# TUMFTM/RadarGNN

Hardware: AMD Instinct MI355X
Metric: radar frames/sec (graph-build + GNN fwd) (higher is better)
Workload: dtype f32 (dense layers: fp32 operands split into 2 f16 terms after an exact power-of-two pre-scale, 3 f16 MFMA products per fp32 product, fp32 accumulate -- more accurate than fp32 MFMA against float64, tests/test_gpu_f16x2.py; RGNN_NO_F16X2=1 selects 3 bf16 terms / 6 products, RGNN_LINEAR_FP32=1 v_mfma_; 1 GPU; C2: per GPU 64 RadarScenes-shaped frames x 3000 pts, radius graph r=1.0, node feats [rcs,velocity_vector,time_index,degree], edge feats [relative_position], 4-layer MPNNConv [224,224,128,64] + emb MLPs + both heads, train-mode BatchNorm, max aggr; frames_per_gpu=64, points_per_gpu=192000, edges_per_gpu=799078, ranks_in_process_group=1

## Files before the change

### include/rgnn.h

```cpp
#ifndef RGNN_H
#define RGNN_H

#include <stdint.h>

#ifdef __cplusplus
extern "C" {
#endif

typedef void* rgnn_stream_t;

#define RGNN_OK 0
#define RGNN_ERR_INVALID_ARGUMENT (-1)
#define RGNN_ERR_LAUNCH (-2)
#define RGNN_ERR_UNSUPPORTED (-3)

#define RGNN_STATUS_KNN_TOO_FEW_POINTS 1
#define RGNN_STATUS_DOT_PRODUCT 2
#define RGNN_STATUS_TIME_INDEX_OVERFLOW 4
#define RGNN_STATUS_EDGE_COUNT_CHANGED 8
#define RGNN_STATUS_NOT_SYMMETRIC 16
#define RGNN_STATUS_SPLITK_TIMEOUT 32
#define RGNN_STATUS_GT_OBJECT_TOO_LARGE 64
#define RGNN_STATUS_GT_DEGENERATE_OBJECT 128
#define RGNN_STATUS_PREPROCESS_BAD_ROW 256
// ... 120 lines not shown
int rgnn_radius_counts(const int32_t* deg, int64_t n, const int32_t* rowptr, int32_t threshold, int32_t* out2, rgnn_stream_t stream);

#define RGNN_STAT_ROWS 4
#define RGNN_AFFINE_ROWS 3
typedef struct rgnn_linear_args {
  const float* A1; int64_t lda1; int32_t k1;
  const float* A2; int64_t lda2; int32_t k2;
  const float* W1; const float* W2; int64_t ldw; int32_t w_split;
  const float* bias1; const float* bias2;
  const float* residual; int64_t ldr;
  float* out; int64_t ldo;
  int64_t m; int32_t n;
  int32_t relu_out;
  float* col_stats;
  const int32_t* row_index;
  const int64_t* m_dev;
  int32_t accumulate;
  int32_t gather_only;
  const int32_t* residual_index;
  const void* W_planes;
  int32_t w_planes_kp;
  void* splitk_ws;
  int64_t splitk_ws_bytes;
  const float* a1_scale_shift;
  int32_t a1_relu;
  int32_t relu_from_col;
  const void* W_planes_f16;
  const float* a1_bound;
  const float* a2_bound;
  float* out_absmax;
  const int32_t* a1_panel_segment;
} rgnn_linear_args;
#define RGNN_BOUND_SLOTS 256
enum { RGNN_LINEAR_PATH_OTHER = 0, RGNN_LINEAR_PATH_DMA_BF16X3 = 1, RGNN_LINEAR_PATH_DMA_F16X2 = 2 };
int32_t rgnn_linear_fwd_path(const rgnn_linear_args* args );
int64_t rgnn_linear_planes_f16_bytes(int32_t n, int32_t k);
int rgnn_linear_split_weights_f16(const float* W1, const float* W2, int64_t ldw, int32_t w_split, int32_t n, int32_t k,
                                  void* planes , rgnn_stream_t stream);
int32_t rgnn_linear_fwd_fuses_a1_affine(const rgnn_linear_args* args );
enum { RGNN_LINEAR_FAMILY_NONE = 0, RGNN_LINEAR_FAMILY_TINY = 1, RGNN_LINEAR_FAMILY_FP32 = 2, RGNN_LINEAR_FAMILY_X3 = 3,
       RGNN_LINEAR_FAMILY_DMA = 4 };
void rgnn_linear_fwd_plan(const rgnn_linear_args* args , int32_t out[8] );
int64_t rgnn_linear_splitk_ws_bytes(void);
int64_t rgnn_linear_stat_panels(int64_t m);
int32_t rgnn_linear_planes_kp(int32_t k);
int rgnn_linear_split_weights(const float* W1, const float* W2, int64_t ldw, int32_t w_split, int32_t n, int32_t k,
                              void* planes , rgnn_stream_t stream);
int rgnn_linear_fwd(const rgnn_linear_args* args , rgnn_stream_t stream);

int32_t rgnn_embed3_supported(int32_t k0, int32_t n1, int32_t n2, int32_t n3);
int rgnn_embed3(const float* x, int64_t ldx, int32_t k0, const float* W1, int64_t ldw1, const float* b1, int32_t n1,
                const void* W2_planes_f16, const float* b2, int32_t n2, const void* W3_planes_f16, const float* b3, int32_t n3,
                int32_t relu3, int64_t m, float* out, int64_t ldo, float* out_absmax, rgnn_stream_t stream);
int rgnn_tiny_mlp2(const float* A, int64_t lda, int32_t k0, const int32_t* row_index , int64_t m,
                   const float* W1, int64_t ldw1, const float* b1, int32_t n1, int32_t relu1, const float* W2, int64_t ldw2,
                   const float* b2, int32_t n2, int32_t relu2, float* out, int64_t ldo, rgnn_stream_t stream);

int rgnn_batchnorm_finalize(const float* stats_a, int64_t panels_a, const int64_t* rows_a ,
                            const float* stats_b , int64_t panels_b, const int64_t* rows_b ,
                            int64_t m, int32_t n, const float* gamma, const float* beta, float* running_mean,
                            float* running_var, int64_t* num_batches_tracked, int32_t training, float momentum, float eps,
                            float* scale_shift , const float* in_bound ,
                            float* out_bound , rgnn_stream_t stream);
int rgnn_batchnorm_segments(const float* x, int64_t ldx, const int64_t* seg_ptr , int64_t n_seg, int32_t n,
                            const float* gamma, const float* beta, float* running_mean, float* running_var,
                            int64_t* num_batches_tracked, float momentum, float eps, double* seg_sums, float* table,
                            const float* in_bound, float* out_bound, rgnn_stream_t stream);
int rgnn_batchnorm_act_segments(const float* x, int64_t ldx, const int64_t* seg_ptr, int64_t n_seg, int32_t n, const float* gamma,
                                const float* beta, float* running_mean, float* running_var, int64_t* num_batches_tracked,
                                float momentum, float eps, int32_t relu, double* seg_sums, float* table, float* y, int64_t ldy,
                                const float* in_bound, float* out_bound, rgnn_stream_t stream);
int rgnn_batchnorm_segments_from_panels(const float* stats_a, const int32_t* panel_start_a, const float* stats_b,
                                        const int32_t* panel_start_b, const int64_t* seg_ptr, int64_t n_seg, int32_t n,
                                        const float* gamma, const float* beta, float* running_mean, float* running_var,
                                        int64_t* num_batches_tracked, float momentum, float eps, double* seg_sums, float* table,
                                        const float* in_bound, float* out_bound, rgnn_stream_t stream);
int rgnn_pad_list_by_segment(const int32_t* list, const int64_t* count, const int64_t* seg_ptr, int64_t n_seg, int32_t* out_list,
                             int64_t* out_count, int32_t* tile_segment, int32_t* stat_panel_start, rgnn_stream_t stream);
int rgnn_pad_list_pair_by_segment(const int32_t* list_a, const int64_t* count_a, const int32_t* list_b, const int64_t* count_b,
                                  const int64_t* seg_ptr, int64_t n_seg, int32_t* out_list_a, int64_t* out_count_a,
                                  int32_t* tile_segment_a, int32_t* stat_panel_start_a, int32_t* out_list_b, int64_t* out_count_b,
                                  int32_t* tile_segment_b, int32_t* stat_panel_start_b, rgnn_stream_t stream);
int rgnn_scale_shift_act_segments(const float* x, int64_t ldx, const float* table, const int64_t* seg_ptr, int64_t n_seg,
                                  int64_t m, int32_t n, int32_t relu, float* y, int64_t ldy, rgnn_stream_t stream);
int rgnn_column_stats(const float* x, int64_t ldx, int64_t m, int32_t n, float* col_stats ,
                      rgnn_stream_t stream);
int rgnn_scale_shift_act(const float* x, int64_t ldx, const float* scale_shift, int64_t m, int32_t n, int32_t relu,
                         float* y, int64_t ldy, rgnn_stream_t stream);

#define RGNN_AGGR_MAX 0
#define RGNN_AGGR_MEAN 1
#define RGNN_AGGR_ADD 2
#define RGNN_AGGR_MIN 3
#define RGNN_AGGR_VAR 4
#define RGNN_AGGR_STD 5
#define RGNN_MPNN_SKIP_EMPTY_ROWS 1
int rgnn_mpnn_aggregate(const float* P, int64_t ldp, const float* p_bias, const float* Q, int64_t ldq,
                        const float* We , int64_t ldwe, const float* edge_attr_sorted,
                        int32_t de, const int32_t* rowptr_t, const int32_t* src_sorted,
                        const int32_t* node_order ,
                        const int32_t* chunk_start , int32_t n_chunks, int64_t n,
                        int32_t d, int32_t aggr, float* out, int64_t ldo, int32_t flags, float* out_absmax ,
                        rgnn_stream_t stream);
int rgnn_mpnn_aggregate_max_arg(const float* p_bias, const float* Q, int64_t ldq, const float* We, int64_t ldwe,
                                const float* edge_attr_sorted, int32_t de, const int32_t* rowptr_t, const int32_t* src_sorted,
                                const int32_t* node_order, const int32_t* chunk_start, int32_t n_chunks, int64_t n, int32_t d,
// ... 230 lines not shown
```

### radargnn_amd/_lib.py

```python
from __future__ import annotations

import ctypes as C
import os

import torch

_HERE = os.path.dirname(os.path.abspath(__file__))
LIB_PATH = os.environ.get("RGNN_LIB") or os.path.join(_HERE, "librgnn.so")

c_i32, c_i64, c_f32, c_f64, c_vp = C.c_int32, C.c_int64, C.c_float, C.c_double, C.c_void_p


class RgnnGrid(C.Structure):
    _fields_ = [("X", c_vp), ("dim", c_i32), ("n", c_i64), ("frame_ptr", c_vp), ("n_frames", c_i64),
                ("ws", c_vp), ("ws_bytes", c_i64)]


class RgnnLinearArgs(C.Structure):
    _fields_ = [("A1", c_vp), ("lda1", c_i64), ("k1", c_i32),
                ("A2", c_vp), ("lda2", c_i64), ("k2", c_i32),
                ("W1", c_vp), ("W2", c_vp), ("ldw", c_i64), ("w_split", c_i32),
                ("bias1", c_vp), ("bias2", c_vp),
                ("residual", c_vp), ("ldr", c_i64),
                ("out", c_vp), ("ldo", c_i64),
                ("m", c_i64), ("n", c_i32),
                ("relu_out", c_i32),
                ("col_stats", c_vp),
                ("row_index", c_vp), ("m_dev", c_vp), ("accumulate", c_i32), ("gather_only", c_i32),
                ("residual_index", c_vp),
                ("W_planes", c_vp), ("w_planes_kp", c_i32),
                ("splitk_ws", c_vp), ("splitk_ws_bytes", c_i64),
                ("a1_scale_shift", c_vp), ("a1_relu", c_i32), ("relu_from_col", c_i32),
                ("W_planes_f16", c_vp), ("a1_bound", c_vp), ("a2_bound", c_vp), ("out_absmax", c_vp), ("a1_panel_segment", c_vp)]


class RgnnEvalBoxes(C.Structure):
    _fields_ = [("translation", c_vp), ("size", c_vp), ("rotation", c_vp), ("velocity", c_vp), ("name", c_vp), ("attribute", c_vp),
                ("keep", c_vp), ("ptr", c_vp), ("n", c_i64)]


SIGNATURES = {
    "rgnn_version": (C.c_char_p, []),
    "rgnn_last_error": (C.c_char_p, []),
    "rgnn_env_reload": (None, []),
    "rgnn_profile_next_launch": (None, [c_vp, c_vp]),
    "rgnn_stream_create": (c_i32, [C.POINTER(c_vp)]),
    "rgnn_stream_destroy": (c_i32, [c_vp]),
    "rgnn_scan_tmp_bytes": (c_i64, [c_i64]),
    "rgnn_exclusive_scan_i32": (c_i32, [c_vp, c_vp, c_i64, c_vp, c_vp]),
    "rgnn_grid_workspace_bytes": (c_i64, [c_i64, c_i64, c_i32]),
    "rgnn_grid_build": (c_i32, [C.POINTER(RgnnGrid), c_f64, c_f64, c_i64, c_vp]),
    "rgnn_grid_order_offsets": (c_i32, [c_i64, c_i64, c_i32, C.POINTER(c_i64), C.POINTER(c_i64)]),
    "rgnn_radius_graph_count": (c_i32, [C.POINTER(RgnnGrid), c_f64, c_vp, c_vp]),
    "rgnn_radius_graph_fill": (c_i32, [C.POINTER(RgnnGrid), c_f64, c_vp, c_vp, c_vp, c_i64, c_vp, c_vp, c_vp]),
    "rgnn_radius_graph_rows": (c_i32, [C.POINTER(RgnnGrid), c_f64, c_vp, c_vp, c_vp, c_i64, c_vp, c_vp, c_vp, c_i32, c_vp]),
    "rgnn_radius_graph_rows_direct": (c_i32, [C.POINTER(RgnnGrid), c_f64, c_vp, c_vp, c_vp, c_i64, c_vp, c_vp, c_vp, c_i32, c_vp]),
    "rgnn_radius_rows_commit": (c_i32, [c_vp, c_i64, c_i64, c_vp, c_vp, c_vp, c_vp, c_vp]),
    "rgnn_knn_graph": (c_i32, [C.POINTER(RgnnGrid), c_i32, c_i64, c_vp, c_vp, c_vp, c_vp, c_i32, c_vp, c_vp]),
    "rgnn_knn_degree_from_csr": (c_i32, [c_vp, c_vp, c_vp, c_vp, c_i64, c_i32, c_vp, c_vp]),
    "rgnn_undirected_degree_preset": (c_i32, [c_vp, c_vp, c_i64, c_vp, c_vp]),
    "rgnn_grid_cell_order": (c_i32, [C.POINTER(RgnnGrid), c_vp, c_vp]),
    "rgnn_undirected_degree": (c_i32, [c_vp, c_vp, c_i64, c_vp, c_vp]),
    "rgnn_csr_by_target_tmp_bytes": (c_i64, [c_i64, c_i64]),
    "rgnn_invert_permutation": (c_i32, [c_vp, c_i64, c_vp, c_vp]),
    "rgnn_source_rowptr": (c_i32, [c_vp, c_i64, c_i64, c_vp, c_vp, c_vp, c_vp]),
    "rgnn_csr_by_target": (c_i32, [c_vp, c_i64, c_i64, c_vp, c_vp, c_vp, c_vp, c_vp, c_i32, c_vp]),
    "rgnn_csr_by_target_frames": (c_i32, [c_vp, c_i64, c_i64, c_i64, c_vp, c_i64, c_i64, c_vp, c_vp, c_vp, c_vp, c_vp, c_vp, c_vp, c_vp]),
    "rgnn_csr_by_target_symmetric": (c_i32, [c_vp, c_vp, c_i64, c_i64, c_vp, c_vp, c_vp, c_vp, c_vp, c_vp, c_vp, c_vp]),
    "rgnn_embed3_supported": (c_i32, [c_i32, c_i32, c_i32, c_i32]),
    "rgnn_embed3": (c_i32, [c_vp, c_i64, c_i32, c_vp, c_i64, c_vp, c_i32, c_vp, c_vp, c_i32, c_vp, c_vp, c_i32, c_i32, c_i64, c_vp, c_i64,
                            c_vp, c_vp]),
    "rgnn_edge_features": (c_i32, [c_vp, c_vp, c_vp, c_i64, C.POINTER(c_i32), c_i32, c_i32, c_vp, c_i32, c_vp, c_vp]),
    "rgnn_edge_features_reversed": (c_i32, [c_vp, c_vp, c_vp, c_i64, c_vp, c_i64, C.POINTER(c_i32), c_i32, c_i32, c_vp, c_i32, c_vp, c_vp]),
    "rgnn_node_features": (c_i32, [c_vp, c_vp, c_vp, c_vp, c_vp, c_i64, C.POINTER(c_i32), c_i32, c_vp, c_i32, c_vp]),
    "rgnn_node_features_time_index": (c_i32, [c_vp, c_vp, c_vp, c_vp, c_vp, c_i64, c_vp, c_i64, C.POINTER(c_i32), c_i32, c_vp, c_i32,
                                              c_vp, c_vp, c_vp]),
    "rgnn_split_by_degree_frames": (c_i32, [c_vp, c_vp, c_i64, c_vp, c_vp, c_vp, c_vp, c_vp, c_vp, c_vp]),
    "rgnn_radius_counts": (c_i32, [c_vp, c_i64, c_vp, c_i32, c_vp, c_vp]),
    "rgnn_time_index": (c_i32, [c_vp, c_vp, c_i64, c_vp, c_vp, c_vp]),
    "rgnn_time_index_ws_bytes": (c_i64, [c_i64]),
    "rgnn_time_index_ws": (c_i32, [c_vp, c_vp, c_i64, c_i64, c_vp, c_vp, c_vp, c_i64, c_vp]),
    "rgnn_linear_stat_panels": (c_i64, [c_i64]),
    "rgnn_linear_fwd": (c_i32, [C.POINTER(RgnnLinearArgs), c_vp]),
    "rgnn_linear_fwd_fuses_a1_affine": (c_i32, [C.POINTER(RgnnLinearArgs)]),
    "rgnn_linear_fwd_plan": (None, [C.POINTER(RgnnLinearArgs), C.POINTER(c_i32 * 8)]),
    "rgnn_linear_planes_kp": (c_i32, [c_i32]),
    "rgnn_linear_fwd_path": (c_i32, [C.POINTER(RgnnLinearArgs)]),
    "rgnn_linear_planes_f16_bytes": (c_i64, [c_i32, c_i32]),
    "rgnn_linear_split_weights_f16": (c_i32, [c_vp, c_vp, c_i64, c_i32, c_i32, c_i32, c_vp, c_vp]),
    "rgnn_linear_splitk_ws_bytes": (c_i64, []),
    "rgnn_linear_split_weights": (c_i32, [c_vp, c_vp, c_i64, c_i32, c_i32, c_i32, c_vp, c_vp]),
    "rgnn_tiny_mlp2": (c_i32, [c_vp, c_i64, c_i32, c_vp, c_i64, c_vp, c_i64, c_vp, c_i32, c_i32, c_vp, c_i64, c_vp, c_i32, c_i32, c_vp,
                       c_i64, c_vp]),
    "rgnn_batchnorm_finalize": (c_i32, [c_vp, c_i64, c_vp, c_vp, c_i64, c_vp, c_i64, c_i32, c_vp, c_vp, c_vp, c_vp, c_vp, c_i32, c_f32,
                                        c_f32, c_vp, c_vp, c_vp, c_vp]),
    "rgnn_batchnorm_segments": (c_i32, [c_vp, c_i64, c_vp, c_i64, c_i32, c_vp, c_vp, c_vp, c_vp, c_vp, c_f32, c_f32, c_vp, c_vp,
                                        c_vp, c_vp, c_vp]),
    "rgnn_batchnorm_act_segments": (c_i32, [c_vp, c_i64, c_vp, c_i64, c_i32, c_vp, c_vp, c_vp, c_vp, c_vp, c_f32, c_f32, c_i32, c_vp,
                                            c_vp, c_vp, c_i64, c_vp, c_vp, c_vp]),
    "rgnn_batchnorm_segments_from_panels": (c_i32, [c_vp, c_vp, c_vp, c_vp, c_vp, c_i64, c_i32, c_vp, c_vp, c_vp, c_vp, c_vp, c_f32,
                                                    c_f32, c_vp, c_vp, c_vp, c_vp, c_vp]),
    "rgnn_pad_list_by_segment": (c_i32, [c_vp, c_vp, c_vp, c_i64, c_vp, c_vp, c_vp, c_vp, c_vp]),
    "rgnn_pad_list_pair_by_segment": (c_i32, [c_vp, c_vp, c_vp, c_vp, c_vp, c_i64, c_vp, c_vp, c_vp, c_vp, c_vp, c_vp, c_vp, c_vp, c_vp]),
    "rgnn_scale_shift_act_segments": (c_i32, [c_vp, c_i64, c_vp, c_vp, c_i64, c_i64, c_i32, c_i32, c_vp, c_i64, c_vp]),
    "rgnn_column_stats": (c_i32, [c_vp, c_i64, c_i64, c_i32, c_vp, c_vp]),
    "rgnn_scale_shift_act": (c_i32, [c_vp, c_i64, c_vp, c_i64, c_i32, c_i32, c_vp, c_i64, c_vp]),
    "rgnn_mpnn_aggregate": (c_i32, [c_vp, c_i64, c_vp, c_vp, c_i64, c_vp, c_i64, c_vp, c_i32, c_vp, c_vp, c_vp, c_vp, c_i32, c_i64,
                                    c_i32, c_i32, c_vp, c_i64, c_i32, c_vp, c_vp]),
    "rgnn_mpnn_aggregate_max_arg": (c_i32, [c_vp, c_vp, c_i64, c_vp, c_i64, c_vp, c_i32, c_vp, c_vp, c_vp, c_vp, c_i32, c_i64, c_i32,
                                            c_vp, c_i64, c_vp, c_i32, C.POINTER(c_i32), c_vp, c_vp]),
    "rgnn_mpnn_win_plan_ints": (c_i64, [c_i64, c_i64]),
    "rgnn_mpnn_win_plan_counters": (None, [c_i64, c_i64, C.POINTER(c_i64), C.POINTER(c_i64)]),
    "rgnn_mpnn_win_plan": (c_i32, [c_vp, c_vp, c_vp, c_i64, c_i64, c_vp, c_vp]),
    "rgnn_mpnn_aggregate_win": (c_i32, [c_vp, c_vp, c_i64, c_vp, c_i64, c_vp, c_i32, c_vp, c_vp, c_vp, c_vp, c_i64, c_i64, c_i32, c_vp,
                                        c_i64, c_i32, c_vp, c_vp, c_vp]),
    "rgnn_mpnn_win_wplanes_bytes": (c_i64, [c_i32]),
    "rgnn_mpnn_win_wplanes": (c_i32, [c_vp, c_i64, c_i32, c_i32, c_vp, c_vp, c_vp]),
    "rgnn_empty_targets": (c_i32, [c_vp, c_vp, c_i64, c_vp, c_vp, c_vp, c_vp, c_vp, c_vp, c_vp]),
    "rgnn_split_targets": (c_i32, [c_vp, c_vp, c_i64, c_vp, c_vp, c_vp, c_vp, c_vp, c_vp, c_vp, c_vp, c_vp]),
    "rgnn_split_targets_by_node": (c_i32, [c_vp, c_vp, c_i64, c_vp, c_vp, c_vp, c_vp, c_vp, c_vp, c_vp, c_vp, c_vp]),
    "rgnn_mpnn_num_chunks": (c_i32, [c_i64, c_i64]),
    "rgnn_mpnn_work_units": (c_i32, [c_i64, c_i64]),
    "rgnn_mpnn_target_weight": (c_i32, [c_i64, c_i64]),
    "rgnn_mpnn_partition": (c_i32, [c_vp, c_i64, c_i64, c_vp, c_vp]),
# ... 105 lines not shown
```

### radargnn_amd/csrc/embed.hip

```cpp
#include "linear_common.h"

namespace {

typedef short raw16x8 __attribute__((ext_vector_type(8)));
constexpr int EM_THREADS = 512, EM_ROWS = 256;

__device__ __forceinline__ float wave_max(float v) {
#pragma unroll
  for (int o = 32; o > 0; o >>= 1) v = fmaxf(v, __shfl_xor(v, o, 64));
  return v;
}
__device__ __forceinline__ void prescale_of(float bound, float& a_mul, float& inv) {
  const int be = (int)((__float_as_uint(bound) >> 23) & 255u);
  int se = 268 - be;
  se = se > 253 ? 253 : se;
  a_mul = __uint_as_float((unsigned)se << 23);
  inv = __uint_as_float((unsigned)(254 - se) << 23);
}
__device__ __forceinline__ void split8(const float (&x)[8], float mul, raw16x8& h, raw16x8& l) {
  f16x8_t hh, ll;
#pragma unroll
  for (int i = 0; i < 8; i++) {
    const float v = x[i] * mul;
    const _Float16 a = (_Float16)v;
// ... 91 lines not shown
        my_stage[((r & 3) + 8 * (r >> 2) + 4 * half) * LDS2 + col] = v;
      }
    }
    m2 = wave_max(m2);
    float mul2, inv2;
    prescale_of(m2, mul2, inv2);
    __builtin_amdgcn_fence(__ATOMIC_ACQ_REL, "wavefront");
    __builtin_amdgcn_wave_barrier();
    f32x16 acc3[T3];
#pragma unroll
    for (int j = 0; j < T3; j++)
#pragma unroll
      for (int r = 0; r < 16; r++) acc3[j][r] = 0.f;
#pragma unroll
    for (int ks = 0; ks < KS3; ks++) {
      const float4 x0 = *(const float4*)(my_stage + (lane & 31) * LDS2 + 16 * ks + 8 * half);
      const float4 x1 = *(const float4*)(my_stage + (lane & 31) * LDS2 + 16 * ks + 8 * half + 4);
      const float xs[8] = {x0.x, x0.y, x0.z, x0.w, x1.x, x1.y, x1.z, x1.w};
      raw16x8 ah, al;
      split8(xs, mul2, ah, al);
#pragma unroll
      for (int j = 0; j < T3; j++) {
        const int col = j * 32 + (lane & 31);
        const raw16x8 bh = *(const raw16x8*)(p3s + ((ks * 2 + 0) * N3 + col) * 16 + 8 * half);
        const raw16x8 bl = *(const raw16x8*)(p3s + ((ks * 2 + 1) * N3 + col) * 16 + 8 * half);
        acc3[j] = mm3(ah, al, bh, bl, acc3[j]);
      }
    }
    __builtin_amdgcn_fence(__ATOMIC_ACQ_REL, "wavefront");
    __builtin_amdgcn_wave_barrier();
    const float o3 = inv2 * w3_inv;
#pragma unroll
    for (int j = 0; j < T3; j++) {
      const int col = j * 32 + (lane & 31);
      const float bb = b3s[col];
#pragma unroll
      for (int r = 0; r < 16; r++) {
        float v = acc3[j][r] * o3 + bb;
        if (relu3) v = fmaxf(v, 0.f);
        const int64_t orow = row0 + (r & 3) + 8 * (r >> 2) + 4 * half;
        if (orow < m) {
          out[orow * ldo + col] = v;
          amax = fmaxf(amax, fabsf(v));
        }
      }
    }
  }
  if (out_absmax != nullptr) {
    amax = wave_max(amax);
    if (lane == 0) bound_raise(out_absmax, blockIdx.x * 8 + wave, amax);
  }
}

}

extern "C" int32_t rgnn_embed3_supported(int32_t k0, int32_t n1, int32_t n2, int32_t n3) {
  return (k0 >= 1 && k0 <= 8 && n1 == 32 && n2 == 64 && n3 == 128) ? 1 : 0;
}

extern "C" int rgnn_embed3(const float* x, int64_t ldx, int32_t k0, const float* W1, int64_t ldw1, const float* b1, int32_t n1,
                           const void* W2_planes_f16, const float* b2, int32_t n2, const void* W3_planes_f16, const float* b3,
                           int32_t n3, int32_t relu3, int64_t m, float* out, int64_t ldo, float* out_absmax, rgnn_stream_t stream) {
  RGNN_CHECK_ARG(m >= 0, "negative m");
  if (m == 0) return RGNN_OK;
  RGNN_CHECK_ARG(rgnn_embed3_supported(k0, n1, n2, n3), "rgnn_embed3 takes <= 8 inputs and layers of 32, 64 and 128 columns");
  RGNN_CHECK_ARG(x && W1 && W2_planes_f16 && W3_planes_f16 && out, "null pointers");
  constexpr int N1 = 32, N2 = 64, N3 = 128;
  const size_t lds = (size_t)(N1 * 9 + N2 + N3) * 4 + (size_t)(N1 / 16 * 2 * N2 * 16 + N2 / 16 * 2 * N3 * 16) * 2 + (size_t)8 * 32 * (N2 + 4) * 4;
  static RgnnOncePerDevice attr_once;
  if (attr_once.first()) {
    hipFuncSetAttribute((const void*)k_embed3<N1, N2, N3>, hipFuncAttributeMaxDynamicSharedMemorySize, (int)lds);
  }
  const int64_t tiles = (m + EM_ROWS - 1) / EM_ROWS;
  const unsigned grid = (unsigned)(tiles < 256 ? tiles : 256);
  hipLaunchKernelGGL((k_embed3<N1, N2, N3>), dim3(grid), dim3(EM_THREADS), lds, (hipStream_t)stream, x, ldx, k0, W1, ldw1, b1,
                     (const _Float16*)W2_planes_f16, b2, (const _Float16*)W3_planes_f16, b3, relu3, m, out, ldo, out_absmax);
  RGNN_CHECK_LAUNCH();
  return RGNN_OK;
}
```

### radargnn_amd/csrc/mpnn_tiles.hip

```cpp
#include "common.h"
#include <stdlib.h>
#include <type_traits>

namespace {

constexpr int MT_THREADS = 256;
constexpr int MT_WAVES = MT_THREADS / 64;
constexpr int MT_QUEUE_INTS = 8 * 16;

typedef float mt_f32x16 __attribute__((ext_vector_type(16)));
typedef __bf16 mt_bf16x8 __attribute__((ext_vector_type(8)));
typedef unsigned int mt_u32x4 __attribute__((ext_vector_type(4)));

__global__ __launch_bounds__(256) void k_tiles_zero_empty(const int32_t* __restrict__ rowptr, const int32_t* __restrict__ order,
                                                         int64_t n, int d, float* __restrict__ out, int64_t ldo) {
  const int lane = threadIdx.x & 63;
  const int64_t p = (int64_t)blockIdx.x * MT_WAVES + (threadIdx.x >> 6);
  if (p >= n || rowptr[p + 1] != rowptr[p]) return;
  const int64_t node = order ? order[p] : p;
  for (int c = lane; c < d; c += 64) out[node * ldo + c] = 0.f;
}

__device__ __forceinline__ void mt_split3(float x, unsigned& t1, unsigned& t2, unsigned& t3) {
  t1 = __float_as_uint(x) & 0xffff0000u;
// ... 275 lines not shown
            }
          }
        }
      }
    };
    float amax_full = 0.f;
    for (int ct = 0; ct < p.n_ct; ct++) {
      const bool partial = AMAX && (ct + 1) * 32 > p.d;
      if (partial) { amax_full = amax; amax = 0.f; }
      if ((gp + ct) & 1) tile_pass(ct, std::integral_constant<int, 1>());
      else tile_pass(ct, std::integral_constant<int, 0>());
      if (partial) amax = fmaxf(amax_full, (ct * 32 + col < p.d) ? amax : 0.f);
    }
    if (p.n_ct < 2) {
      asm volatile("s_waitcnt vmcnt(0)" ::: "memory");
      __syncthreads();
    }
    gp = (gp + p.n_ct) & 1;
    win = nxt; up ^= 1; staged = staged_next;
  }
  if (AMAX) {
#pragma unroll
    for (int o = 32; o > 0; o >>= 1) amax = fmaxf(amax, __shfl_xor(amax, o, 64));
    if (lane == 0)
      atomicMax((unsigned int*)p.out_absmax + ((blockIdx.x * 4 + wave) & (RGNN_BOUND_SLOTS - 1)), __float_as_uint(amax));
  }
}

constexpr int WN_BIG = 64;

constexpr int WN_SEG = 512;
struct WinPlanLayout {
  int n_win, n_seg;
  int64_t off_assign, off_segcnt, off_segbase, off_wend, off_pdeg, off_wstart, off_left, off_leftcnt, off_queue, off_misc, off_tgt, off_eid, off_lrow, off_urow,
      off_wplanes, total_ints;
};
WinPlanLayout win_layout(int64_t n, int64_t n_edges) {
  WinPlanLayout L;
  L.n_seg = (int)((n + WN_SEG - 1) / WN_SEG);
  L.n_win = (int)((n_edges + 3 * n) / 256 + L.n_seg + 2);
  int64_t o = 16;
  auto take = [&](int64_t ints) { const int64_t at = o; o = (o + ints + 15) / 16 * 16; return at; };
  L.off_assign = take(n + 1); L.off_segcnt = take(L.n_seg + 1); L.off_segbase = take(L.n_seg + 2);
  L.off_wend = take(L.n_win + 1);
  L.off_pdeg = take(n + 1); L.off_wstart = take(L.n_win + 1); L.off_left = take(n + 1); L.off_leftcnt = take(4);
  L.off_queue = take(MT_QUEUE_INTS); L.off_misc = take(16 * (int64_t)L.n_win);
  L.off_tgt = take(8 * WN_GPS * (int64_t)L.n_win); L.off_eid = take(512 * (int64_t)L.n_win); L.off_lrow = take(128 * (int64_t)L.n_win);
  L.off_urow = take(WN_UMAX * (int64_t)L.n_win); L.off_wplanes = take(16 * 64 * 32);
  L.total_ints = o;
  return L;
}

__global__ __launch_bounds__(256) void k_win_pdeg(const int32_t* __restrict__ rowptr, int64_t n, int32_t* __restrict__ pdeg,
                                                 int32_t* __restrict__ left, int32_t* __restrict__ leftcnt, int32_t* __restrict__ queue) {
  const int64_t p = (int64_t)blockIdx.x * blockDim.x + threadIdx.x;
  if (p < MT_QUEUE_INTS) queue[p] = 0;
  if (p > n) return;
  if (p == n) { pdeg[p] = 0; return; }
  const int d = rowptr[p + 1] - rowptr[p];
  const int pd = (d + WN_PAD - 1) & ~(WN_PAD - 1);
  if (pd > WN_BIG) left[atomicAdd(leftcnt, 1)] = (int32_t)p;
  pdeg[p] = (pd > WN_BIG) ? 0 : pd;
}
__global__ __launch_bounds__(64) void k_win_greedy(const int32_t* __restrict__ pdeg, int64_t n, int32_t* __restrict__ assign,
                                                  int32_t* __restrict__ segcnt) {
  __shared__ int spd[WN_SEG];
  __shared__ int sas[WN_SEG];
  const int seg = blockIdx.x, lane = threadIdx.x;
  const int64_t p0 = (int64_t)seg * WN_SEG;
  const int cnt = (int)min((int64_t)WN_SEG, n - p0);
  for (int i = lane; i < cnt; i += 64) spd[i] = pdeg[p0 + i];
  __syncthreads();
  {
    int fill = 0;
    int win = 0, any = 0;
    for (int ib = 0; ib < cnt; ib += 64) {
      const int mine_pd = (ib + lane < cnt) ? spd[ib + lane] : 0;
      int mine_as = -1;
      const int nb = min(64, cnt - ib);
      for (int j = 0; j < nb; j++) {
        const int pd = __builtin_amdgcn_readlane(mine_pd, j);
        if (pd == 0) continue;
        const unsigned long long fits = __ballot(lane < 8 && fill + pd <= 64);
        int b = 0;
        if (fits == 0) { win++; fill = 0; }
        else b = __builtin_ctzll(fits);
        const int off = __builtin_amdgcn_readlane(fill, b);
        if (lane == b) fill += pd;
        any = 1;
        if (lane == j) mine_as = (win << 16) | (b * 64 + off);
      }
      if (ib + lane < cnt) sas[ib + lane] = mine_as;
    }
    if (lane == 0) segcnt[seg] = any ? win + 1 : 0;
  }
  __syncthreads();
  for (int i = lane; i < cnt; i += 64) assign[p0 + i] = sas[i];
}
__global__ __launch_bounds__(1024) void k_win_segbase(const int32_t* __restrict__ segcnt, int n_seg, int32_t* __restrict__ segbase) {
  __shared__ int part[1024];
  const int t = threadIdx.x;
  const int per = (n_seg + 1023) / 1024;
  int sum = 0;
  for (int i = t * per; i < min(n_seg, (t + 1) * per); i++) sum += segcnt[i];
  part[t] = sum;
  __syncthreads();
  for (int o = 1; o < 1024; o <<= 1) {
    const int v = t >= o ? part[t - o] : 0;
    __syncthreads();
// ... 171 lines not shown
            for (int j = 0; j < 2; j++) v[u][j] = ok[j] ? Q[r + 64 * j] : 0.f;
          }
#pragma unroll
          for (int u = 0; u < 8; u++) {
            float z[8];
#pragma unroll
            for (int k = 0; k < 8; k++) z[k] = __builtin_bit_cast(float, __builtin_amdgcn_readlane(__builtin_bit_cast(int, my_z[k]), jj[u]));
#pragma unroll
            for (int j = 0; j < 2; j++) {
#pragma unroll
              for (int k = 0; k < 8; k++) v[u][j] = __builtin_fmaf(w[j][k], z[k], v[u][j]);
              m[j] = fmaxf(m[j], v[u][j]);
            }
          }
        }
      }
#pragma unroll
      for (int j = 0; j < 2; j++) {
        if (!ok[j]) continue;
        const int c = cw + 64 * j + lane;
        const float o = m[j] + (p_bias ? p_bias[c] : 0.f);
        out[node * ldo + c] = o;
        amax = fmaxf(amax, fabsf(o));
      }
    }
  }
  if (out_absmax != nullptr) {
#pragma unroll
    for (int o = 32; o > 0; o >>= 1) amax = fmaxf(amax, __shfl_xor(amax, o, 64));
    if (lane == 0 && amax > 0.f)
      atomicMax((unsigned int*)out_absmax + ((blockIdx.x * 4 + wv) & (RGNN_BOUND_SLOTS - 1)), __float_as_uint(amax));
  }
}

}

extern "C" int64_t rgnn_mpnn_win_plan_ints(int64_t n, int64_t n_edges) { return win_layout(n, n_edges).total_ints; }
extern "C" void rgnn_mpnn_win_plan_counters(int64_t n, int64_t n_edges, int64_t* leftover_word, int64_t* windows_word) {
  const WinPlanLayout L = win_layout(n, n_edges);
  *leftover_word = L.off_leftcnt;
  *windows_word = L.off_segbase + L.n_seg;
}

extern "C" int rgnn_mpnn_win_plan(const int32_t* rowptr_t, const int32_t* src_sorted, const int32_t* node_order, int64_t n, int64_t n_edges,
                                  int32_t* plan, rgnn_stream_t stream) {
  RGNN_CHECK_ARG(rowptr_t && plan && n >= 0 && n_edges >= 0, "bad arguments");
  RGNN_CHECK_ARG(n_edges == 0 || src_sorted, "null src_sorted");
  RGNN_CHECK_ARG((((uintptr_t)plan) & 15) == 0, "plan must be 16-byte aligned");
  if (n == 0) return RGNN_OK;
  const WinPlanLayout L = win_layout(n, n_edges);
  hipStream_t s = (hipStream_t)stream;
  hipMemsetAsync(plan + L.off_leftcnt, 0, 16, s);
  hipLaunchKernelGGL(k_win_pdeg, dim3(rgnn_blocks(n + 1 > MT_QUEUE_INTS ? n + 1 : MT_QUEUE_INTS, 256)), dim3(256), 0, s, rowptr_t, n, plan + L.off_pdeg,
                     plan + L.off_left, plan + L.off_leftcnt, plan + L.off_queue);
  hipMemsetAsync(plan + L.off_wend, 0, 4 * (size_t)(L.n_win + 1), s);
  hipLaunchKernelGGL(k_win_greedy, dim3(L.n_seg), dim3(64), 0, s, (const int32_t*)(plan + L.off_pdeg), n, plan + L.off_assign, plan + L.off_segcnt);
  hipLaunchKernelGGL(k_win_segbase, dim3(1), dim3(1024), 0, s, (const int32_t*)(plan + L.off_segcnt), L.n_seg, plan + L.off_segbase);
  hipLaunchKernelGGL(k_win_starts, dim3(rgnn_blocks(n, 256)), dim3(256), 0, s, (const int32_t*)(plan + L.off_assign),
                     (const int32_t*)(plan + L.off_segbase), n, L.n_seg, L.n_win, plan + L.off_wstart, plan + L.off_wend);
  hipLaunchKernelGGL(k_win_pack, dim3(rgnn_blocks(L.n_win, 4)), dim3(256), 0, s, rowptr_t, src_sorted, node_order,
                     (const int32_t*)(plan + L.off_pdeg), (const int32_t*)(plan + L.off_assign), (const int32_t*)(plan + L.off_segbase),
                     (const int32_t*)(plan + L.off_wstart), (const int32_t*)(plan + L.off_wend), L.n_win, plan + L.off_misc,
                     plan + L.off_tgt, plan + L.off_eid, (uint8_t*)(plan + L.off_lrow),
                     plan + L.off_urow, plan + L.off_left, plan + L.off_leftcnt);
  RGNN_CHECK_LAUNCH();
  return RGNN_OK;
}

extern "C" int64_t rgnn_mpnn_win_wplanes_bytes(int32_t d) { return d < 1 ? -1 : (int64_t)((d + 31) / 32) * WN_BBUF; }

extern "C" int rgnn_mpnn_win_wplanes(const float* We, int64_t ldwe, int32_t de, int32_t d, const float* p_bias, void* planes,
                                     rgnn_stream_t stream) {
  RGNN_CHECK_ARG(planes && d >= 1 && de >= 0 && de <= 8 && (de == 0 || We) && (((uintptr_t)planes) & 15) == 0, "bad arguments");
  const int n_ct = (d + 31) / 32;
  hipLaunchKernelGGL(k_win_wplanes, dim3(rgnn_blocks(n_ct * 32, 256)), dim3(256), 0, (hipStream_t)stream, We, (int)ldwe, de, d, n_ct, p_bias,
                     (mt_u32x4*)planes);
  RGNN_CHECK_LAUNCH();
  return RGNN_OK;
}

extern "C" int rgnn_mpnn_aggregate_win(const float* p_bias, const float* Q, int64_t ldq, const float* We, int64_t ldwe,
                                       const float* edge_attr_sorted, int32_t de, const int32_t* rowptr_t, const int32_t* src_sorted,
                                       const int32_t* node_order, int32_t* plan, int64_t n, int64_t n_edges, int32_t d, float* out,
                                       int64_t ldo, int32_t flags, float* out_absmax, const void* wplanes, rgnn_stream_t stream) {
  if (n == 0) return RGNN_OK;
  RGNN_CHECK_ARG(Q && rowptr_t && plan && out && d >= 1, "bad arguments");
  RGNN_CHECK_ARG((flags & ~RGNN_MPNN_SKIP_EMPTY_ROWS) == 0, "unknown flags");
  RGNN_CHECK_ARG(de == 0 || ((We || wplanes) && edge_attr_sorted), "edge attributes given without weights");
  RGNN_CHECK_ARG((((uintptr_t)wplanes) & 15) == 0, "operand image not 16-byte aligned");
  const int64_t q_bytes = ((n - 1) * ldq + d) * 4, o_bytes = ((n - 1) * ldo + d) * 4;
  if (de > 8 || d > 2048 || n >= ((int64_t)1 << 24) || ldq * 4 >= ((int64_t)1 << 24) || q_bytes >= ((int64_t)1 << 31) ||
      o_bytes >= ((int64_t)1 << 31) || (ldq % 4) != 0 || (((uintptr_t)Q) & 15) != 0 || win_layout(n, n_edges).total_ints * 4 >= ((int64_t)1 << 31)) {
    rgnn_set_error("rgnn_mpnn_aggregate_win: shape not covered (de %d, d %d, n %lld, ldq %lld)", de, d, (long long)n, (long long)ldq);
    return RGNN_ERR_UNSUPPORTED;
  }
  hipStream_t s = (hipStream_t)stream;
  if (!(flags & RGNN_MPNN_SKIP_EMPTY_ROWS))
    hipLaunchKernelGGL(k_tiles_zero_empty, dim3(rgnn_blocks(n, MT_WAVES)), dim3(256), 0, s, rowptr_t, node_order, n, d, out, ldo);
  if (n_edges > 0) {
    const WinPlanLayout L = win_layout(n, n_edges);
    WinParams p;
    p.p_bias = p_bias; p.Q = Q; p.ldq4 = (int)(ldq * 4); p.q_bytes = (int)q_bytes;
    p.wplanes = wplanes ? (const mt_u32x4*)wplanes : (const mt_u32x4*)(plan + L.off_wplanes); p.ea = edge_attr_sorted; p.de = de;
    p.ea_vec = (de == 8 && (((uintptr_t)edge_attr_sorted) & 15) == 0) ? 1 : 0;
    p.n_win = L.n_win; p.n_win_dev = plan + L.off_segbase + L.n_seg;
    p.plan = plan; p.plan_bytes = (int)(L.total_ints * 4);
    p.off_misc = (int)(L.off_misc * 4); p.off_eid = (int)(L.off_eid * 4); p.off_lrow = (int)(L.off_lrow * 4); p.off_urow = (int)(L.off_urow * 4); p.off_tgt = (int)(L.off_tgt * 4);
    p.queue = plan + L.off_queue;
// ... 26 lines not shown
```

### radargnn_amd/gnn/gnn_models.py

```python
from __future__ import annotations

from typing import List

import torch
from torch import nn
from torch.nn import ModuleList, ReLU, Sequential

from .. import derived, ops
from .configs import GNNArchitectureConfig
from . import autograd as AG
from .linear import BatchNorm, Linear, frame_scope, run_mlp
from .mpnn_layers import DeferredEdgeAttr, MPNNConv, RadarPointGNNConv, TargetCSR, UnsortedEdgeAttr
from . import linear as _lin_mod


class _rows_of:

    def __init__(self, kind: str):
        self.kind, self.ctx = kind, None

    def __enter__(self):
        if _lin_mod.current_frame_scope() is not None:
            self.ctx = _lin_mod.current_frame_scope().rows_of(self.kind)
            self.ctx.__enter__()
# ... 176 lines not shown
            elif bn.uses_frame_scope():
                h, _ = conv.forward_sorted(x, graph, ea, want_stats=False, edge_tail=edge_tail, x_affine=pending,
                                           **({"x_tail": node_tail} if node_tail is not None else {}))
                node_tail = None
                with _rows_of("node"):
                    x, pending = bn.apply_frames(h, relu=True), None
            else:
                h, stats = conv.forward_sorted(x, graph, ea, want_stats=use_batch, edge_tail=edge_tail, x_affine=pending,
                                               **({"x_tail": node_tail} if node_tail is not None else {}))
                node_tail = None
                x, pending = h, bn.scale_shift(stats, h.shape[0], in_bound=ops.bound_of(h))
        if pending is not None and frames is not None:
            x, pending = ops.scale_shift_act_segments(x, pending, _lin.current_frame_scope().node_ptr, True), None
        if pending is not None:
            fused = self._fused_heads(x, pending) if FUSE_HEADS else None
            if fused is not None:
                return fused
            x = ops.scale_shift_act(x, pending, relu=True)
        with _rows_of("node"):
            c, _ = run_mlp(self.classification_head, x)
            bb, _ = run_mlp(self.regression_head, x)
        return c, bb

    def _frames_fusable(self, x, graph, node_tail) -> bool:
        from . import linear as _lin
        f = _lin.current_frame_scope().node_ptr.numel() - 1
        if f < 1 or x.shape[0] < 256 * f:
            return False
        return all(conv.frames_fusable(x, graph, k1=x.shape[1] if (i == 0 and node_tail is not None) else None)
                   for i, conv in enumerate(self.convs))

    @staticmethod
    def _embedding_front(mods, x: torch.Tensor) -> torch.Tensor:
        if (FUSE_EMBED3 and not AG.is_recording() and len(mods) == 6 and all(isinstance(mods[i], Linear) for i in (0, 2, 4))
                and all(isinstance(mods[i], ReLU) for i in (1, 3, 5)) and x.shape[0] > 0):
            d = lambda t: None if t is None else t.detach()
            l1, l2, l3 = mods[0], mods[2], mods[4]
            out = ops.embed3(x, d(l1.weight), d(l1.bias), d(l2.weight), d(l2.bias), d(l3.weight), d(l3.bias), True)
            if out is not None:
                return out
        return run_mlp(mods, x)[0]

    def _negated(self, w: torch.Tensor) -> torch.Tensor:
        return derived.get(self, "neg", (w,), lambda: (-w.detach()).contiguous())

    @staticmethod
    def _tiny_edge_hidden(hidden) -> bool:
        return (not AG.is_recording() and len(hidden) == 4 and isinstance(hidden[0], Linear) and isinstance(hidden[1], ReLU)
                and isinstance(hidden[2], Linear) and isinstance(hidden[3], ReLU) and hidden[0].in_channels <= 8
                and hidden[0].out_channels <= 8 and hidden[2].out_channels <= 16
                and __import__("os").environ.get("RGNN_NO_TINY_MLP2") is None)

    def _fused_heads(self, h: torch.Tensor, scale_shift: torch.Tensor):
        heads = []
        for seq in (self.classification_head, self.regression_head):
            mods = list(seq)
            if not mods or not isinstance(mods[0], Linear) or (len(mods) > 1 and not isinstance(mods[1], (ReLU, Linear))):
                return None
            relu = len(mods) > 1 and isinstance(mods[1], ReLU)
            heads.append((mods[0], relu, mods[2:] if relu else mods[1:]))
        order = (0, 1) if heads[0][1] <= heads[1][1] else (1, 0)
        first, second = heads[order[0]], heads[order[1]]
        lins = (first[0], second[0])
        if any(l.bias is None for l in lins):
            return None
        n0, n1 = lins[0].weight.shape[0], lins[1].weight.shape[0]
        pad = (-n0) % 4
        def build():
            w0, b0 = lins[0].weight.detach(), lins[0].bias.detach()
            return (torch.cat([w0, w0.new_zeros((pad, w0.shape[1])), lins[1].weight.detach()], 0).contiguous(),
                    torch.cat([b0, b0.new_zeros(pad), lins[1].bias.detach()], 0).contiguous())
        w, b = derived.get(self, "heads", (lins[0].weight, lins[0].bias, lins[1].weight, lins[1].bias), build)
        relu_any = first[1] or second[1]
        out = ops.linear(h, w, b, relu=relu_any, relu_from=0 if first[1] else n0 + pad, a1_affine=scale_shift, a1_relu=True)
        res = [None, None]
        for which, (_, _, rest), view in ((order[0], first, out[:, :n0]), (order[1], second, out[:, n0 + pad:n0 + pad + n1])):
            res[which] = run_mlp(rest, view)[0] if rest else view
        return res[0], res[1]
```

### radargnn_amd/ops.py

```python
from __future__ import annotations

import ctypes as C
import math
import os
import sys
from typing import List, Optional, Sequence, Tuple

import torch

from . import _lib, derived
from ._lib import RgnnError, RgnnGrid, RgnnLinearArgs, check, lib

EDGE_FEATURE_CODES = {
    "point_pair_features": 0, "spatial_euclidean_distance": 1, "velocity_euclidean_distance": 2,
    "relative_position": 3, "relative_velocity": 4,
}
EDGE_FEATURE_WIDTH = {"point_pair_features": 4, "spatial_euclidean_distance": 1, "velocity_euclidean_distance": 1,
                      "relative_position": 2, "relative_velocity": 2}
NODE_FEATURE_CODES = {"rcs": 0, "time_index": 1, "degree": 2, "velocity_vector_length": 3, "velocity_vector": 4,
                      "spatial_coordinates": 5}
NODE_FEATURE_WIDTH = {"rcs": 1, "time_index": 1, "degree": 1, "velocity_vector_length": 1, "velocity_vector": 2,
                      "spatial_coordinates": 2}
AGGR_CODES = {"max": 0, "mean": 1, "add": 2, "sum": 2, "min": 3, "var": 4, "std": 5}
SHIFT_INVARIANT_AGGR = ("var", "std")
# ... 801 lines not shown
            raise RgnnError("this launch cannot apply per-segment scale / shift tables (not on the LDS-DMA kernel)")
        COUNTERS["fused_a1_affine_segments"] = COUNTERS.get("fused_a1_affine_segments", 0) + 1
    elif a1_affine is not None:
        a1_affine = _dev(a1_affine, "a1_affine", torch.float32).contiguous()
        if a1_affine.shape != (AFFINE_ROWS, k1):
            raise ValueError("a1_affine must be [AFFINE_ROWS, k1]")
        args, dma, f16 = prepare(a1, a1_affine)
        if FUSE_A1_AFFINE and lib.rgnn_linear_fwd_fuses_a1_affine(C.byref(args)):
            COUNTERS["fused_a1_affine"] += 1
        else:
            args, dma, f16 = prepare(scale_shift_act(a1, a1_affine, relu=a1_relu), None)
    else:
        args, dma, f16 = prepare(a1, None)
    if (padded_row_list or a1_affine_tiles is not None) and not dma:
        raise RgnnError("a segment-padded row list needs the LDS-DMA kernel, which this launch does not qualify for")
    word = None
    if (track and dma
            and not (row_index is not None and getattr(out, "_rgnn_rows_without_bound", False))):
        word = bound_of(out) if row_index is not None else None
        if word is None:
            word = ctx().bounds.word()
        args.out_absmax = _ptr(word)
    tok = ctx().profiler.begin("linear") if ctx().profiler is not None else None
    check(lib.rgnn_linear_fwd(C.byref(args), _stream()))
    set_bound(out, word)
    if row_index is not None and word is None:
        out._rgnn_rows_without_bound = True
    elif row_index is None and hasattr(out, "_rgnn_rows_without_bound"):
        del out._rgnn_rows_without_bound
    COUNTERS["f16x2" if f16 else "other_dense"] = COUNTERS.get("f16x2" if f16 else "other_dense", 0) + 1
    if tok is not None:
        ctx().profiler.end(tok, m=m if m_dev is None else m_dev, n=n, k=k1 + k2, x3=planes is not None, f16=f16)
    return (out, stats) if (want_stats or stats_out is not None) else out


def embed3(x: torch.Tensor, w1, b1, w2, b2, w3, b3, relu3: bool) -> Optional[torch.Tensor]:
    x = _rowmajor(_dev(x, "x", torch.float32), "x")
    if not lib.rgnn_embed3_supported(x.shape[1], w1.shape[0], w2.shape[0], w3.shape[0]):
        return None
    if w1.shape[1] != x.shape[1] or w2.shape[1] != w1.shape[0] or w3.shape[1] != w2.shape[0]:
        raise ValueError("layer widths do not chain")
    w1 = _rowmajor(_dev(w1, "w1", torch.float32), "w1")
    p2 = weight_planes_f16(w2, None, w2.shape[1])
    p3 = weight_planes_f16(w3, None, w3.shape[1])
    m = x.shape[0]
    out = torch.empty((m, w3.shape[0]), dtype=torch.float32, device=x.device)
    word = ctx().bounds.word() if ctx().bounds is not None else None
    check(lib.rgnn_embed3(_ptr(x), _ld(x), x.shape[1], _ptr(w1), _ld(w1), _ptr(b1), w1.shape[0], _ptr(p2), _ptr(b2), w2.shape[0],
                          _ptr(p3), _ptr(b3), w3.shape[0], 1 if relu3 else 0, m, _ptr(out), _ld(out), _ptr(word), _stream()))
    set_bound(out, word)
    return out


def tiny_mlp2(a: torch.Tensor, row_index: Optional[torch.Tensor], w1, b1, relu1: bool, w2, b2, relu2: bool) -> torch.Tensor:
    a = _rowmajor(_dev(a, "a", torch.float32), "a")
    w1 = _rowmajor(_dev(w1, "w1", torch.float32), "w1"); w2 = _rowmajor(_dev(w2, "w2", torch.float32), "w2")
    m = a.shape[0] if row_index is None else row_index.numel()
    if row_index is not None:
        _dev(row_index, "row_index", torch.int32)
    out = torch.empty((m, w2.shape[0]), dtype=torch.float32, device=a.device)
    check(lib.rgnn_tiny_mlp2(_ptr(a), _ld(a), a.shape[1], _ptr(row_index), m, _ptr(w1), _ld(w1), _ptr(b1), w1.shape[0],
                             1 if relu1 else 0, _ptr(w2), _ld(w2), _ptr(b2), w2.shape[0], 1 if relu2 else 0, _ptr(out),
                             _ld(out), _stream()))
    return out


def empty_targets(rowptr_t: torch.Tensor, node_order: Optional[torch.Tensor]):
    _dev(rowptr_t, "rowptr_t", torch.int32)
    n = rowptr_t.numel() - 1
    dev = rowptr_t.device
    flags = torch.empty(max(n, 1), dtype=torch.int32, device=dev)
    pos = torch.empty(n + 1, dtype=torch.int32, device=dev)
    tmp = torch.empty(max(lib.rgnn_scan_tmp_bytes(n), 256), dtype=torch.uint8, device=dev)
    lst = torch.empty(max(n, 1), dtype=torch.int32, device=dev)
    cnt = torch.empty(1, dtype=torch.int64, device=dev)
    slot = torch.empty(max(n, 1), dtype=torch.int32, device=dev)
    check(lib.rgnn_empty_targets(_ptr(rowptr_t), _ptr(node_order), n, _ptr(flags), _ptr(pos), _ptr(tmp), _ptr(lst),
                                 _ptr(cnt), _ptr(slot), _stream()))
    return lst, cnt, slot


SORTED_ROW_LISTS = __import__("os").environ.get("RGNN_VISITING_ORDER_LISTS") is None


def split_targets(rowptr_t: torch.Tensor, node_order: Optional[torch.Tensor], rank: Optional[torch.Tensor] = None,
                  by_node: bool = False):
    _dev(rowptr_t, "rowptr_t", torch.int32)
    n = rowptr_t.numel() - 1
    dev = rowptr_t.device
    flags = torch.empty(max(n, 1), dtype=torch.int32, device=dev)
    pos = torch.empty(n + 1, dtype=torch.int32, device=dev)
    tmp = torch.empty(max(lib.rgnn_scan_tmp_bytes(n), 256), dtype=torch.uint8, device=dev)
    lst = torch.empty(max(n, 1), dtype=torch.int32, device=dev)
    cnt = torch.empty(1, dtype=torch.int64, device=dev)
    slot = torch.empty(max(n, 1), dtype=torch.int32, device=dev)
    lst_ne = torch.empty(max(n, 1), dtype=torch.int32, device=dev)
    cnt_ne = torch.empty(1, dtype=torch.int64, device=dev)
    if by_node and SORTED_ROW_LISTS and (node_order is None or rank is not None):
        if rank is not None:
            _dev(rank, "rank", torch.int32)
        check(lib.rgnn_split_targets_by_node(_ptr(rowptr_t), _ptr(rank), n, _ptr(flags), _ptr(pos), _ptr(tmp), _ptr(lst),
                                             _ptr(cnt), _ptr(slot), _ptr(lst_ne), _ptr(cnt_ne), _stream()))
        return lst, cnt, slot, lst_ne, cnt_ne
    check(lib.rgnn_split_targets(_ptr(rowptr_t), _ptr(node_order), n, _ptr(flags), _ptr(pos), _ptr(tmp), _ptr(lst), _ptr(cnt),
                                 _ptr(slot), _ptr(lst_ne), _ptr(cnt_ne), _stream()))
    return lst, cnt, slot, lst_ne, cnt_ne
# ... 1281 lines not shown
```

Baseline: 33250 frames/s.

## Fuse BatchNorm-ReLU and both prediction heads into one kernel; fold wend memset

```diff
diff --git a/include/rgnn.h b/include/rgnn.h
--- a/include/rgnn.h
+++ b/include/rgnn.h
@@ -196,6 +196,10 @@
 int rgnn_embed3(const float* x, int64_t ldx, int32_t k0, const float* W1, int64_t ldw1, const float* b1, int32_t n1,
                 const void* W2_planes_f16, const float* b2, int32_t n2, const void* W3_planes_f16, const float* b3, int32_t n3,
                 int32_t relu3, int64_t m, float* out, int64_t ldo, float* out_absmax, rgnn_stream_t stream);
+int32_t rgnn_heads_supported(int32_t k, int32_t nc, int32_t nh, int32_t nr);
+int rgnn_heads(const float* h, int64_t ldh, int32_t k, const float* table, const float* Wc, int64_t ldwc, const float* bc, int32_t nc,
+               const float* W1, int64_t ldw1, const float* b1, int32_t nh, const float* W2, int64_t ldw2, const float* b2, int32_t nr,
+               int64_t m, float* cls, int64_t ldc, float* box, int64_t ldb, rgnn_stream_t stream);
 int rgnn_tiny_mlp2(const float* A, int64_t lda, int32_t k0, const int32_t* row_index , int64_t m,
                    const float* W1, int64_t ldw1, const float* b1, int32_t n1, int32_t relu1, const float* W2, int64_t ldw2,
                    const float* b2, int32_t n2, int32_t relu2, float* out, int64_t ldo, rgnn_stream_t stream);
diff --git a/radargnn_amd/_lib.py b/radargnn_amd/_lib.py
--- a/radargnn_amd/_lib.py
+++ b/radargnn_amd/_lib.py
@@ -70,6 +70,9 @@
     "rgnn_embed3_supported": (c_i32, [c_i32, c_i32, c_i32, c_i32]),
     "rgnn_embed3": (c_i32, [c_vp, c_i64, c_i32, c_vp, c_i64, c_vp, c_i32, c_vp, c_vp, c_i32, c_vp, c_vp, c_i32, c_i32, c_i64, c_vp, c_i64,
                             c_vp, c_vp]),
+    "rgnn_heads_supported": (c_i32, [c_i32, c_i32, c_i32, c_i32]),
+    "rgnn_heads": (c_i32, [c_vp, c_i64, c_i32, c_vp, c_vp, c_i64, c_vp, c_i32, c_vp, c_i64, c_vp, c_i32, c_vp, c_i64, c_vp, c_i32, c_i64, c_vp,
+                           c_i64, c_vp, c_i64, c_vp]),
     "rgnn_edge_features": (c_i32, [c_vp, c_vp, c_vp, c_i64, C.POINTER(c_i32), c_i32, c_i32, c_vp, c_i32, c_vp, c_vp]),
     "rgnn_edge_features_reversed": (c_i32, [c_vp, c_vp, c_vp, c_i64, c_vp, c_i64, C.POINTER(c_i32), c_i32, c_i32, c_vp, c_i32, c_vp, c_vp]),
     "rgnn_node_features": (c_i32, [c_vp, c_vp, c_vp, c_vp, c_vp, c_i64, C.POINTER(c_i32), c_i32, c_vp, c_i32, c_vp]),
diff --git a/radargnn_amd/csrc/embed.hip b/radargnn_amd/csrc/embed.hip
--- a/radargnn_amd/csrc/embed.hip
+++ b/radargnn_amd/csrc/embed.hip
@@ -167,6 +167,109 @@
   }
 }
 
+constexpr int HD_THREADS = 256, HD_LD = 33;
+__device__ __forceinline__ constexpr int hd_k(int i) { return (i & ~7) | ((i & 1) << 2) | ((i & 7) >> 1); }
+
+template <int K>
+__global__ __launch_bounds__(HD_THREADS) void k_heads(const float* __restrict__ h, int64_t ldh, const float* __restrict__ table,
+                                                     const float* __restrict__ Wc, int64_t ldwc, const float* __restrict__ bc, int nc,
+                                                     const float* __restrict__ W1, int64_t ldw1, const float* __restrict__ b1, int nh,
+                                                     const float* __restrict__ W2, int64_t ldw2, const float* __restrict__ b2, int nr,
+                                                     int64_t m, float* __restrict__ cls, int64_t ldc, float* __restrict__ box,
+                                                     int64_t ldb) {
+  __shared__ float hd_stage[HD_THREADS / 64][64 * HD_LD];
+  const int lane = threadIdx.x & 63, wave = threadIdx.x >> 6;
+  const int64_t row0 = (int64_t)blockIdx.x * HD_THREADS + wave * 64;
+  if (row0 >= m) return;
+  float* const my = hd_stage[wave];
+  float a[K];
+#pragma unroll
+  for (int hh = 0; hh < K / 32; hh++) {
+    const int c = 32 * hh + 4 * (lane & 7);
+    const float4 mu = *(const float4*)(table + c), sc = *(const float4*)(table + K + c), sh = *(const float4*)(table + 2 * K + c);
+    float4 v[8];
+#pragma unroll
+    for (int j = 0; j < 8; j++) {
+      const int64_t r = row0 + 8 * j + (lane >> 3);
+      v[j] = r < m ? *(const float4*)(h + r * ldh + c) : make_float4(0.f, 0.f, 0.f, 0.f);
+    }
+#pragma unroll
+    for (int j = 0; j < 8; j++) {
+      float* const w = my + (8 * j + (lane >> 3)) * HD_LD + 4 * (lane & 7);
+      w[0] = fmaxf(fmaf(v[j].x - mu.x, sc.x, sh.x), 0.f);
+      w[1] = fmaxf(fmaf(v[j].y - mu.y, sc.y, sh.y), 0.f);
+      w[2] = fmaxf(fmaf(v[j].z - mu.z, sc.z, sh.z), 0.f);
+      w[3] = fmaxf(fmaf(v[j].w - mu.w, sc.w, sh.w), 0.f);
+    }
+    __builtin_amdgcn_fence(__ATOMIC_ACQ_REL, "wavefront");
+    __builtin_amdgcn_wave_barrier();
+#pragma unroll
+    for (int k = 0; k < 32; k++) a[32 * hh + k] = my[lane * HD_LD + k];
+    __builtin_amdgcn_fence(__ATOMIC_ACQ_REL, "wavefront");
+    __builtin_amdgcn_wave_barrier();
+  }
+  const int64_t row = row0 + lane;
+  const bool live = row < m;
+#pragma unroll
+  for (int c = 0; c < 16; c++) {
+    if (c < nc) {
+      float acc = 0.f;
+#pragma unroll
+      for (int i = 0; i < K; i++) acc = fmaf(a[hd_k(i)], Wc[c * ldwc + hd_k(i)], acc);
+      acc += bc ? bc[c] : 0.f;
+      if (live) cls[row * ldc + c] = acc;
+    }
+  }
+  float hid[16];
+#pragma unroll
+  for (int c = 0; c < 16; c++) {
+    float acc = 0.f;
+    if (c < nh) {
+#pragma unroll
+      for (int i = 0; i < K; i++) acc = fmaf(a[hd_k(i)], W1[c * ldw1 + hd_k(i)], acc);
+      acc += b1 ? b1[c] : 0.f;
+      acc = fmaxf(acc, 0.f);
+    }
+    hid[c] = acc;
+  }
+#pragma unroll
+  for (int c = 0; c < 8; c++) {
+    if (c < nr) {
+      float acc = 0.f;
+#pragma unroll
+      for (int i = 0; i < 16; i++)
+        if (hd_k(i) < nh) acc = fmaf(hid[hd_k(i)], W2[c * ldw2 + hd_k(i)], acc);
+      acc += b2 ? b2[c] : 0.f;
+      if (live) box[row * ldb + c] = acc;
+    }
+  }
+}
+
+}
+
+extern "C" int32_t rgnn_heads_supported(int32_t k, int32_t nc, int32_t nh, int32_t nr) {
+  return ((k == 32 || k == 64) && nc >= 1 && nc <= 16 && nh >= 1 && nh <= 16 && nr >= 1 && nr <= 8) ? 1 : 0;
+}
+
+extern "C" int rgnn_heads(const float* h, int64_t ldh, int32_t k, const float* table, const float* Wc, int64_t ldwc, const float* bc,
+                          int32_t nc, const float* W1, int64_t ldw1, const float* b1, int32_t nh, const float* W2, int64_t ldw2,
+                          const float* b2, int32_t nr, int64_t m, float* cls, int64_t ldc, float* box, int64_t ldb,
+                          rgnn_stream_t stream) {
+  RGNN_CHECK_ARG(m >= 0, "negative m");
+  if (m == 0) return RGNN_OK;
+  RGNN_CHECK_ARG(rgnn_heads_supported(k, nc, nh, nr), "rgnn_heads takes 32 or 64 inputs, <= 16 classes, <= 16 hidden and <= 8 box columns");
+  RGNN_CHECK_ARG(h && table && Wc && W1 && W2 && cls && box, "null pointers");
+  RGNN_CHECK_ARG(ldh >= k && ldwc >= k && ldw1 >= k && ldw2 >= nh && ldc >= nc && ldb >= nr, "leading dimension below the row length");
+  RGNN_CHECK_ARG((ldh % 4) == 0 && (((uintptr_t)h) & 15) == 0 && (((uintptr_t)table) & 15) == 0, "h rows and the table must be 16-byte aligned");
+  const unsigned grid = (unsigned)((m + HD_THREADS - 1) / HD_THREADS);
+  if (k == 64)
+    hipLaunchKernelGGL(k_heads<64>, dim3(grid), dim3(HD_THREADS), 0, (hipStream_t)stream, h, ldh, table, Wc, ldwc, bc, nc, W1, ldw1, b1, nh, W2, ldw2,
+                       b2, nr, m, cls, ldc, box, ldb);
+  else
+    hipLaunchKernelGGL(k_heads<32>, dim3(grid), dim3(HD_THREADS), 0, (hipStream_t)stream, h, ldh, table, Wc, ldwc, bc, nc, W1, ldw1, b1, nh, W2, ldw2,
+                       b2, nr, m, cls, ldc, box, ldb);
+  RGNN_CHECK_LAUNCH();
+  return RGNN_OK;
 }
 
 extern "C" int32_t rgnn_embed3_supported(int32_t k0, int32_t n1, int32_t n2, int32_t n3) {
diff --git a/radargnn_amd/csrc/mpnn_tiles.hip b/radargnn_amd/csrc/mpnn_tiles.hip
--- a/radargnn_amd/csrc/mpnn_tiles.hip
+++ b/radargnn_amd/csrc/mpnn_tiles.hip
@@ -351,9 +351,11 @@
 }
 
 __global__ __launch_bounds__(256) void k_win_pdeg(const int32_t* __restrict__ rowptr, int64_t n, int32_t* __restrict__ pdeg,
-                                                 int32_t* __restrict__ left, int32_t* __restrict__ leftcnt, int32_t* __restrict__ queue) {
+                                                 int32_t* __restrict__ left, int32_t* __restrict__ leftcnt, int32_t* __restrict__ queue,
+                                                 int32_t* __restrict__ wend, int n_win) {
   const int64_t p = (int64_t)blockIdx.x * blockDim.x + threadIdx.x;
   if (p < MT_QUEUE_INTS) queue[p] = 0;
+  for (int64_t i = p; i <= n_win; i += (int64_t)gridDim.x * blockDim.x) wend[i] = 0;
   if (p > n) return;
   if (p == n) { pdeg[p] = 0; return; }
   const int d = rowptr[p + 1] - rowptr[p];
@@ -631,8 +633,7 @@
   hipStream_t s = (hipStream_t)stream;
   hipMemsetAsync(plan + L.off_leftcnt, 0, 16, s);
   hipLaunchKernelGGL(k_win_pdeg, dim3(rgnn_blocks(n + 1 > MT_QUEUE_INTS ? n + 1 : MT_QUEUE_INTS, 256)), dim3(256), 0, s, rowptr_t, n, plan + L.off_pdeg,
-                     plan + L.off_left, plan + L.off_leftcnt, plan + L.off_queue);
-  hipMemsetAsync(plan + L.off_wend, 0, 4 * (size_t)(L.n_win + 1), s);
+                     plan + L.off_left, plan + L.off_leftcnt, plan + L.off_queue, plan + L.off_wend, L.n_win);
   hipLaunchKernelGGL(k_win_greedy, dim3(L.n_seg), dim3(64), 0, s, (const int32_t*)(plan + L.off_pdeg), n, plan + L.off_assign, plan + L.off_segcnt);
   hipLaunchKernelGGL(k_win_segbase, dim3(1), dim3(1024), 0, s, (const int32_t*)(plan + L.off_segcnt), L.n_seg, plan + L.off_segbase);
   hipLaunchKernelGGL(k_win_starts, dim3(rgnn_blocks(n, 256)), dim3(256), 0, s, (const int32_t*)(plan + L.off_assign),
diff --git a/radargnn_amd/gnn/gnn_models.py b/radargnn_amd/gnn/gnn_models.py
--- a/radargnn_amd/gnn/gnn_models.py
+++ b/radargnn_amd/gnn/gnn_models.py
@@ -252,6 +252,13 @@
                 and __import__("os").environ.get("RGNN_NO_TINY_MLP2") is None)
 
     def _fused_heads(self, h: torch.Tensor, scale_shift: torch.Tensor):
+        cm, rm = list(self.classification_head), list(self.regression_head)
+        if (not AG.is_recording() and scale_shift.dim() == 2 and len(cm) == 1 and isinstance(cm[0], Linear) and len(rm) == 3
+                and isinstance(rm[0], Linear) and isinstance(rm[1], ReLU) and isinstance(rm[2], Linear) and h.shape[0] > 0):
+            d = lambda t: None if t is None else t.detach()
+            out = ops.heads(h, scale_shift, d(cm[0].weight), d(cm[0].bias), d(rm[0].weight), d(rm[0].bias), d(rm[2].weight), d(rm[2].bias))
+            if out is not None:
+                return out
         heads = []
         for seq in (self.classification_head, self.regression_head):
             mods = list(seq)
diff --git a/radargnn_amd/ops.py b/radargnn_amd/ops.py
--- a/radargnn_amd/ops.py
+++ b/radargnn_amd/ops.py
@@ -877,6 +877,26 @@
     return out
 
 
+def heads(h: torch.Tensor, scale_shift: torch.Tensor, wc, bc, w1, b1, w2, b2):
+    h = _rowmajor(_dev(h, "h", torch.float32), "h")
+    m, k = h.shape
+    if not lib.rgnn_heads_supported(k, wc.shape[0], w1.shape[0], w2.shape[0]):
+        return None
+    if wc.shape[1] != k or w1.shape[1] != k or w2.shape[1] != w1.shape[0]:
+        raise ValueError("layer widths do not chain")
+    if scale_shift.shape != (AFFINE_ROWS, k):
+        raise ValueError("scale_shift must be [AFFINE_ROWS, k]")
+    scale_shift = _dev(scale_shift, "scale_shift", torch.float32).contiguous()
+    if _ld(h) % 4 or h.data_ptr() % 16 or scale_shift.data_ptr() % 16:
+        return None
+    wc, w1, w2 = (_rowmajor(_dev(w, n, torch.float32), n) for w, n in ((wc, "wc"), (w1, "w1"), (w2, "w2")))
+    cls = torch.empty((m, wc.shape[0]), dtype=torch.float32, device=h.device)
+    box = torch.empty((m, w2.shape[0]), dtype=torch.float32, device=h.device)
+    check(lib.rgnn_heads(_ptr(h), _ld(h), k, _ptr(scale_shift), _ptr(wc), _ld(wc), _ptr(bc), wc.shape[0], _ptr(w1), _ld(w1), _ptr(b1),
+                         w1.shape[0], _ptr(w2), _ld(w2), _ptr(b2), w2.shape[0], m, _ptr(cls), _ld(cls), _ptr(box), _ld(box), _stream()))
+    return cls, box
+
+
 def tiny_mlp2(a: torch.Tensor, row_index: Optional[torch.Tensor], w1, b1, relu1: bool, w2, b2, relu2: bool) -> torch.Tensor:
     a = _rowmajor(_dev(a, "a", torch.float32), "a")
     w1 = _rowmajor(_dev(w1, "w1", torch.float32), "w1"); w2 = _rowmajor(_dev(w2, "w2", torch.float32), "w2")
```

Measured after the change: 32690 frames/s. 0.983x the previous value.
